# facebookresearch/localrf

Hardware: AMD Instinct MI355X
Metric: rays/sec (4096-ray batch, 512 samples, 300^3 grid) (higher is better)
Workload: dtype f32 (colour network: split-bf16 3-term products on v_mfma_f32_32x32x16_bf16, fp32 accumulate, <= 3e-5 vs the exact-fp32 engine; gathers and compositing fp32); 1 GPU; configs[1]: single 300^3 TensorVMSplit, 4096 rays x 512 samples per GPU, full density+appearance+MLP render, eval forward; rays_per_gpu=4096, samples_per_ray=512, grid=300, parallelism=ray-shard x1, mlp_engine=bf16x3

## Files before the change

### localrf_amd/csrc/lrf_common.h

```cpp
#pragma once
#include "lrf_tu.h"
#include <hip/hip_runtime.h>
#include <stdint.h>
#include "../../include/lrf.h"

namespace lrf {

constexpr int MAT0[3] = {0, 0, 1};
constexpr int MAT1[3] = {1, 2, 2};
constexpr int VEC[3]  = {2, 1, 0};

constexpr int LRF_CAS = 32;
__host__ __device__ constexpr int app_pc(int c) { return 8 * (c / 6) + c % 6; }

constexpr int IMG_BAS  = 0;
constexpr int IMG_W1   = IMG_BAS + 2 * 3 * 64 * 8;
constexpr int IMG_W2   = IMG_W1 + 8 * 2 * 64 * 4;
constexpr int IMG_W3H  = IMG_W2 + 8 * 8 * 64 * 4;
constexpr int IMG_B1   = IMG_W3H + 4 * 32 * 4;
constexpr int IMG_B2   = IMG_B1 + 128;
constexpr int IMG_W3V  = IMG_B2 + 128;
constexpr int IMG_FLOATS = IMG_W3V + 16;

constexpr int IMGB_BAS = 0;
// ... 42 lines not shown
  L.mlp = off; off = align64(off + IMG_FLOATS);
  L.mlpb = off; off = align64(off + (size_t)IMGB_ALL * 4);
  for (int p = 0; p < 3; ++p) { L.aplane2[p] = off; off = align64(off + (size_t)L.pw[p] * L.ph[p] * LRF_CA); }
  for (int p = 0; p < 3; ++p) { L.aline2[p]  = off; off = align64(off + (size_t)L.ll[p] * LRF_CA); }
  L.mlpw = off; off = align64(off + (size_t)W32_ALL_U4 * 4);
  L.mlpwt = off; off = align64(off + (size_t)W32T_ALL_U4 * 4);
  L.total = off;
  return L;
}

constexpr int ACT_FEAT = 0, ACT_LD = 32;
constexpr int GRD_GO = 0, GRD_DFEAT = 16, GRD_DX = 48, GRD_LD = 128;
static_assert(ACT_FEAT % 16 == 0 && ACT_LD % 16 == 0, "fragment blocks are 16 columns");
static_assert(GRD_DFEAT % 16 == 0 && GRD_DX % 16 == 0 && GRD_LD % 16 == 0 && GRD_LD - GRD_DX == 80, "fragment blocks are 16 columns");
__host__ __device__ inline size_t frag_off(size_t row, int col, int ld) {
  return (row >> 4) * (size_t)(16 * ld) + (size_t)((col >> 4) * 256 + ((((col >> 2) & 3) * 16 + (int)(row & 15)) << 2) + (col & 3));
}
__device__ __forceinline__ float* frag_lane_base(float* buf, size_t tile, int ld, int s, int g) {
  return buf + tile * (size_t)(16 * ld) + ((g * 16 + s) << 2);
}
__device__ __forceinline__ const float* grd_dx_row(const float* grd, size_t row) {
  return grd + (row >> 4) * (size_t)(16 * GRD_LD) + GRD_DX * 16 + (row & 15) * (GRD_LD - GRD_DX);
}
__device__ __forceinline__ const float* grd_dx8(const float* grd, size_t row, int p, int grp) {
  return grd + (row >> 4) * (size_t)(16 * GRD_LD) + GRD_DX * 16 + (((p * 3 + grp) * 16 + (int)(row & 15)) << 3);
}

struct DField {
  const float* dplane[3]; const float* dline[3];
  const float* aplane[3]; const float* aline[3];
  const float* mlp;
  const uint4* mlpb;
  const float* aplane2[3]; const float* aline2[3];
  const uint4* mlpw;
  const uint4* mlpwt;
  int pw[3], ph[3], ll[3];
  const float* alpha_vol; int ax, ay, az;
  float m_lo[3], m_inv[3];
  float lo[3], inv[3];
  float hi[3];
  float density_shift, distance_scale, weight_thres;
  float term_T;
  const float* basis; const float* w1; const float* b1; const float* w2; const float* b2;
  const float* w3; const float* b3;
  int fea_pe, view_pe, fc;
  float* dump;
  float* rdir;
  const int* perm;
};

__device__ __forceinline__ void contract3(float& x, float& y, float& z) {
  float m = fmaxf(fmaxf(fabsf(x), fabsf(y)), fabsf(z));
  m = fmaxf(m, 1e-6f);
  if (m > 1.0f) {
    const float s = (2.0f * m - 1.0f) / (m * m);
    x *= s; y *= s; z *= s;
  }
}

__device__ __forceinline__ void tap1d(float u, int size, int& i0, int& i1, float& t) {
  float ix = ((u + 1.0f) * 0.5f) * (float)(size - 1);
  ix = fminf(fmaxf(ix, 0.0f), (float)(size - 1));
  const float f0 = floorf(ix);
  t = ix - f0;
  i0 = (int)f0;
  i1 = min(i0 + 1, size - 1);
}

struct AxisTaps { int i0[3], i1[3]; float t[3]; };
__device__ __forceinline__ AxisTaps axis_taps(const int pw0, const int ph0, const int ll0, const float u[3]) {
  AxisTaps a;
  tap1d(u[0], pw0, a.i0[0], a.i1[0], a.t[0]);
  tap1d(u[1], ph0, a.i0[1], a.i1[1], a.t[1]);
  tap1d(u[2], ll0, a.i0[2], a.i1[2], a.t[2]);
  return a;
}

__device__ __forceinline__ float feature2density(float f, float shift, bool relu) {
  if (relu) return fmaxf(f, 0.0f);
  const float y = f + shift;
  return y > 20.0f ? y : log1pf(expf(y));
}

__device__ __forceinline__ float alpha_mask_sample(const DField& f, float x, float y, float z) {
  const float ux = (x - f.m_lo[0]) * f.m_inv[0] - 1.0f;
  const float uy = (y - f.m_lo[1]) * f.m_inv[1] - 1.0f;
  const float uz = (z - f.m_lo[2]) * f.m_inv[2] - 1.0f;
  const float ix = ((ux + 1.0f) * 0.5f) * (float)(f.ax - 1);
  const float iy = ((uy + 1.0f) * 0.5f) * (float)(f.ay - 1);
  const float iz = ((uz + 1.0f) * 0.5f) * (float)(f.az - 1);
  const float fx = floorf(ix), fy = floorf(iy), fz = floorf(iz);
  const float tx = ix - fx, ty = iy - fy, tz = iz - fz;
  const int x0 = (int)fx, y0 = (int)fy, z0 = (int)fz;
  float out = 0.0f;
#pragma unroll
  for (int dz = 0; dz < 2; ++dz)
#pragma unroll
    for (int dy = 0; dy < 2; ++dy)
#pragma unroll
      for (int dx = 0; dx < 2; ++dx) {
        const int xi = x0 + dx, yi = y0 + dy, zi = z0 + dz;
        if (xi >= 0 && xi < f.ax && yi >= 0 && yi < f.ay && zi >= 0 && zi < f.az) {
          const float w = (dx ? tx : 1.0f - tx) * (dy ? ty : 1.0f - ty) * (dz ? tz : 1.0f - tz);
          out += f.alpha_vol[((size_t)zi * f.ay + yi) * f.ax + xi] * w;
        }
      }
  return out;
}

__device__ __forceinline__ void sample_point(const DField& f, const float o[3], const float dh[3],
                                             float zk, float x[3], float u[3]) {
  x[0] = o[0] + dh[0] * zk; x[1] = o[1] + dh[1] * zk; x[2] = o[2] + dh[2] * zk;
  contract3(x[0], x[1], x[2]);
#pragma unroll
  for (int a = 0; a < 3; ++a) u[a] = (x[a] - f.lo[a]) * f.inv[a] - 1.0f;
}

__device__ __forceinline__ float4 ld4(const float* p) { return *reinterpret_cast<const float4*>(p); }
__device__ __forceinline__ float2 ld2(const float* p) { return *reinterpret_cast<const float2*>(p); }

__device__ __forceinline__ float density_feature(const DField& f, const float u[3]) {
  float feat = 0.0f;
#pragma unroll
  for (int p = 0; p < 3; ++p) {
    int x0, x1, y0, y1, l0, l1; float tx, ty, tl;
    tap1d(u[MAT0[p]], f.pw[p], x0, x1, tx);
    tap1d(u[MAT1[p]], f.ph[p], y0, y1, ty);
    tap1d(u[VEC[p]],  f.ll[p], l0, l1, tl);
    const float* pl = f.dplane[p];
    const float* q00 = pl + ((size_t)y0 * f.pw[p] + x0) * LRF_CD;
    const float* q10 = pl + ((size_t)y0 * f.pw[p] + x1) * LRF_CD;
    const float* q01 = pl + ((size_t)y1 * f.pw[p] + x0) * LRF_CD;
    const float* q11 = pl + ((size_t)y1 * f.pw[p] + x1) * LRF_CD;
    const float* r0 = f.dline[p] + (size_t)l0 * LRF_CD;
    const float* r1 = f.dline[p] + (size_t)l1 * LRF_CD;
    const float w00 = (1.0f - tx) * (1.0f - ty), w10 = tx * (1.0f - ty);
    const float w01 = (1.0f - tx) * ty,          w11 = tx * ty;
    const float wl0 = 1.0f - tl, wl1 = tl;
    float sp = 0.0f;
#pragma unroll
    for (int h = 0; h < LRF_CD / 4; ++h) {
      const float4 a = ld4(q00 + 4 * h), b = ld4(q10 + 4 * h), c = ld4(q01 + 4 * h), d = ld4(q11 + 4 * h);
      const float4 e = ld4(r0 + 4 * h), g = ld4(r1 + 4 * h);
      sp += (a.x * w00 + b.x * w10 + c.x * w01 + d.x * w11) * (e.x * wl0 + g.x * wl1);
      sp += (a.y * w00 + b.y * w10 + c.y * w01 + d.y * w11) * (e.y * wl0 + g.y * wl1);
      sp += (a.z * w00 + b.z * w10 + c.z * w01 + d.z * w11) * (e.z * wl0 + g.z * wl1);
      sp += (a.w * w00 + b.w * w10 + c.w * w01 + d.w * w11) * (e.w * wl0 + g.w * wl1);
    }
    feat += sp;
  }
  return feat;
}

__device__ __forceinline__ float4 ld4b(const float* base, unsigned byte_off) {
  return *reinterpret_cast<const float4*>(reinterpret_cast<const char*>(base) + byte_off);
}

__device__ __forceinline__ float density_feature32(const DField& f, const float u[3]) {
  float feat = 0.0f;
#pragma unroll
  for (int p = 0; p < 3; ++p) {
    int x0, x1, y0, y1, l0, l1; float tx, ty, tl;
    tap1d(u[MAT0[p]], f.pw[p], x0, x1, tx);
    tap1d(u[MAT1[p]], f.ph[p], y0, y1, ty);
    tap1d(u[VEC[p]],  f.ll[p], l0, l1, tl);
    const unsigned row0 = (unsigned)y0 * (unsigned)f.pw[p], row1 = (unsigned)y1 * (unsigned)f.pw[p];
    const unsigned o00 = (row0 + x0) * (LRF_CD * 4u), o10 = (row0 + x1) * (LRF_CD * 4u);
    const unsigned o01 = (row1 + x0) * (LRF_CD * 4u), o11 = (row1 + x1) * (LRF_CD * 4u);
    const unsigned q0 = (unsigned)l0 * (LRF_CD * 4u), q1 = (unsigned)l1 * (LRF_CD * 4u);
    const float w00 = (1.0f - tx) * (1.0f - ty), w10 = tx * (1.0f - ty);
    const float w01 = (1.0f - tx) * ty,          w11 = tx * ty;
    const float wl0 = 1.0f - tl, wl1 = tl;
    float sp = 0.0f;
#pragma unroll
    for (int h = 0; h < LRF_CD / 4; ++h) {
      const float4 a = ld4b(f.dplane[p], o00 + 16 * h), b = ld4b(f.dplane[p], o10 + 16 * h);
      const float4 c = ld4b(f.dplane[p], o01 + 16 * h), d = ld4b(f.dplane[p], o11 + 16 * h);
      const float4 e = ld4b(f.dline[p], q0 + 16 * h), g = ld4b(f.dline[p], q1 + 16 * h);
      sp += (a.x * w00 + b.x * w10 + c.x * w01 + d.x * w11) * (e.x * wl0 + g.x * wl1);
      sp += (a.y * w00 + b.y * w10 + c.y * w01 + d.y * w11) * (e.y * wl0 + g.y * wl1);
      sp += (a.z * w00 + b.z * w10 + c.z * w01 + d.z * w11) * (e.z * wl0 + g.z * wl1);
      sp += (a.w * w00 + b.w * w10 + c.w * w01 + d.w * w11) * (e.w * wl0 + g.w * wl1);
    }
    feat += sp;
  }
  return feat;
}

typedef float f32x2 __attribute__((ext_vector_type(2)));
template <bool LDSL>
__device__ __forceinline__ float density_feature_m(const DField& f, const float u[3], const float* const s_line[3]) {
  f32x2 acc = {0.0f, 0.0f};
  const AxisTaps at = axis_taps(f.pw[0], f.ph[0], f.ll[0], u);
#pragma unroll
  for (int p = 0; p < 3; ++p) {
    const int x0 = at.i0[MAT0[p]], x1 = at.i1[MAT0[p]], y0 = at.i0[MAT1[p]], y1 = at.i1[MAT1[p]];
    const int l0 = at.i0[VEC[p]], l1 = at.i1[VEC[p]];
    const float tx = at.t[MAT0[p]], ty = at.t[MAT1[p]], tl = at.t[VEC[p]];
    const unsigned row0 = (unsigned)y0 * (unsigned)f.pw[p], row1 = (unsigned)y1 * (unsigned)f.pw[p];
    const unsigned o00 = (row0 + x0) * (LRF_CD * 4u), o10 = (row0 + x1) * (LRF_CD * 4u);
    const unsigned o01 = (row1 + x0) * (LRF_CD * 4u), o11 = (row1 + x1) * (LRF_CD * 4u);
    const f32x2 w00 = {(1.0f - tx) * (1.0f - ty), (1.0f - tx) * (1.0f - ty)}, w10 = {tx * (1.0f - ty), tx * (1.0f - ty)};
    const f32x2 w01 = {(1.0f - tx) * ty, (1.0f - tx) * ty}, w11 = {tx * ty, tx * ty};
    const f32x2 wl0 = {1.0f - tl, 1.0f - tl}, wl1 = {tl, tl};
#pragma unroll
    for (int h = 0; h < LRF_CD / 4; ++h) {
      const float4 a = ld4b(f.dplane[p], o00 + 16 * h), b = ld4b(f.dplane[p], o10 + 16 * h);
      const float4 c = ld4b(f.dplane[p], o01 + 16 * h), d = ld4b(f.dplane[p], o11 + 16 * h);
      float4 e, g;
      if (LDSL) {
        e = *reinterpret_cast<const float4*>(s_line[p] + l0 * LRF_CD + 4 * h);
        g = *reinterpret_cast<const float4*>(s_line[p] + l1 * LRF_CD + 4 * h);
      } else {
        e = ld4b(f.dline[p], (unsigned)l0 * (LRF_CD * 4u) + 16 * h);
        g = ld4b(f.dline[p], (unsigned)l1 * (LRF_CD * 4u) + 16 * h);
      }
      const f32x2 a0 = {a.x, a.y}, a1 = {a.z, a.w}, b0 = {b.x, b.y}, b1 = {b.z, b.w};
      const f32x2 c0 = {c.x, c.y}, c1 = {c.z, c.w}, d0 = {d.x, d.y}, d1 = {d.z, d.w};
      const f32x2 e0 = {e.x, e.y}, e1 = {e.z, e.w}, g0 = {g.x, g.y}, g1 = {g.z, g.w};
      acc += (a0 * w00 + b0 * w10 + c0 * w01 + d0 * w11) * (e0 * wl0 + g0 * wl1);
      acc += (a1 * w00 + b1 * w10 + c1 * w01 + d1 * w11) * (e1 * wl0 + g1 * wl1);
    }
  }
  return acc.x + acc.y;
}

__device__ __forceinline__ void wave_scan_prod(float v, int lane, float& excl, float& total) {
  float p = v;
#pragma unroll
  for (int d = 1; d < 64; d <<= 1) {
    const float t = __shfl_up(p, d, 64);
    if (lane >= d) p *= t;
  }
  excl = __shfl_up(p, 1, 64);
  if (lane == 0) excl = 1.0f;
  total = __shfl(p, 63, 64);
}

__device__ __forceinline__ float wave_sum(float v) {
#pragma unroll
  for (int d = 32; d >= 1; d >>= 1) v += __shfl_xor(v, d, 64);
  return v;
}

}
```

### localrf_amd/csrc/lrf_render.hip

```cpp
#include <hip/hip_runtime.h>
#include <stdint.h>
#include <stdio.h>
#include <string.h>
#include <stdlib.h>
#include <mutex>
#include "lrf_common.h"

namespace lrf {

constexpr int ITEM = 16;

thread_local char g_err[512] = "";
static int set_err(const char* msg, hipError_t e = hipSuccess) {
  char* slot = lrf_error_slot();
  if (e != hipSuccess) snprintf(slot, 512, "%s: %s", msg, hipGetErrorString(e));
  else snprintf(slot, 512, "%s", msg);
  return 1;
}
#define LRF_HIP(call) do { hipError_t e_ = (call); if (e_ != hipSuccess) return set_err(#call, e_); } while (0)

struct PackSeg { const float* src; float* dst; int C, H, W, CS, app; };
struct PackTab { PackSeg s[18]; };
struct PackMlp { float* mlp; uint32_t* mlpb; uint32_t* mlpw; uint32_t* mlpwt; int mode; };
__device__ void pack_mlp_elem(const LrfParams& p, float* __restrict__ img, int idx);
// ... 116 lines not shown
    return;
  }
  const int u4 = idx >> 2, wj = idx & 3;
  const int lane = u4 & 63, part = (u4 >> 6) & 1, frag = u4 >> 7;
  const int i = lane & 15, g = lane >> 4;
  unsigned short out[2];
#pragma unroll
  for (int h = 0; h < 2; ++h) {
    const int j = 2 * wj + h;
    float v = 0.0f;
    if (frag < 6) {
      const int t1 = frag / 3, pl = frag % 3, row = 16 * t1 + i;
      if (j < 6 && row < LRF_APP_DIM) v = p.basis[row * 72 + pl * LRF_CA + 6 * g + j];
    } else if (frag < 14) {
      const int t1 = frag - 6;
      const int col = 16 * (j >> 2) + 4 * g + (j & 3);
      if (col < LRF_APP_DIM) v = p.w1[(16 * t1 + i) * LRF_APP_DIM + col];
    } else {
      const int t1 = (frag - 14) >> 2, ks = (frag - 14) & 3;
      const int col = 16 * (2 * ks + (j >> 2)) + 4 * g + (j & 3);
      v = p.w2[(16 * t1 + i) * LRF_FEATC + col];
    }
    const unsigned short hi = bf16_bits(v);
    out[h] = part ? bf16_bits(v - bf16_val(hi)) : hi;
  }
  img[idx] = (uint32_t)out[0] | ((uint32_t)out[1] << 16);
}

__device__ void pack_mlp_w32_elem(const LrfParams& p, uint32_t* __restrict__ img, int idx) {
  if (idx >= W32_ALL_U4 * 4) return;
  if (idx >= W32_U4 * 4) {
    const int e = idx - W32_U4 * 4;
    float v = 0.0f;
    if (e < W32_T_B2) v = p.b1[e - W32_T_B1];
    else if (e < W32_T_W3) v = p.b2[e - W32_T_B2];
    else if (e < W32_T_B3) {
      const int c = (e - W32_T_W3) / W32_T_W3_LD, u = (e - W32_T_W3) % W32_T_W3_LD;
      if (u < LRF_FEATC + 3) v = p.w3[c * (LRF_FEATC + 3) + u];
    } else if (e < W32_T_B3 + 3) v = p.b3[e - W32_T_B3];
    img[idx] = __float_as_uint(v);
    return;
  }
  const int u4 = idx >> 2, wj = idx & 3;
  const int lane = u4 & 63, part = (u4 >> 6) & 1, frag = u4 >> 7;
  const int n = lane & 31, h = lane >> 5;
  unsigned short out[2];
#pragma unroll
  for (int hh = 0; hh < 2; ++hh) {
    const int j = 2 * wj + hh;
    float v = 0.0f;
    if (frag < W32_W1) {
      const int c = w32_chan(h, 8 * frag + j);
      if (c >= 0 && n < LRF_APP_DIM) v = p.basis[n * 72 + c];
    } else if (frag < W32_W2) {
      const int e = frag - W32_W1, m = e >> 1, q = e & 1;
      const int u = w32_unit(0, q, h, j);
      if (u < LRF_APP_DIM) v = p.w1[(32 * m + n) * LRF_APP_DIM + u];
    } else {
      const int e = frag - W32_W2, m = e >> 3, m0 = (e >> 1) & 3, q = e & 1;
      v = p.w2[(32 * m + n) * LRF_FEATC + w32_unit(m0, q, h, j)];
    }
    const unsigned short hi = bf16_bits(v);
    out[hh] = part ? bf16_bits(v - bf16_val(hi)) : hi;
  }
  img[idx] = (uint32_t)out[0] | ((uint32_t)out[1] << 16);
}

constexpr int LRF_MULTI_MAX = 4;
struct MultiF { DField f[LRF_MULTI_MAX]; int nf, Rf, Rs, lo; };
__device__ __forceinline__ int multi_io(const MultiF& m, int k, int vray) { return k * m.Rs + m.lo + (vray - k * m.Rf); }
template <bool MULTI> struct FieldArg { typedef DField type; };
template <> struct FieldArg<true> { typedef MultiF type; };
__device__ __forceinline__ const DField& field_of(const DField& f, int) { return f; }
__device__ __forceinline__ const DField& field_of(const MultiF& m, int k) { return m.f[k]; }

template <bool LDSL, bool MULTI = false>
__global__ __launch_bounds__(1024) void k_march(
    typename FieldArg<MULTI>::type fin, const float* __restrict__ rays, const float* __restrict__ z, int R, int S,
    uint32_t flags, float floater,
    float* __restrict__ depth, float* __restrict__ acc_ws, float* __restrict__ w_all,
    int* __restrict__ ncomp, uint16_t* __restrict__ cidx, float* __restrict__ cw,
    float* __restrict__ feat_out ) {
  extern __shared__ float s_alpha_all[];
  const int wave = threadIdx.x >> 6, lane = threadIdx.x & 63;
  const int nb = gridDim.x;
  const int lb = (nb % 8 == 0) ? (int)(blockIdx.x % 8) * (nb / 8) + (int)(blockIdx.x / 8) : (int)blockIdx.x;
  const int nw = blockDim.x >> 6;
  const int ray = lb * nw + wave;
  int fk_ = 0;
  if constexpr (MULTI) fk_ = min((lb * nw) / fin.Rf, fin.nf - 1);
  const DField& f = field_of(fin, fk_);
  int io_ray = ray;
  if constexpr (MULTI) io_ray = multi_io(fin, fk_, ray);
  const float* s_line[3] = {nullptr, nullptr, nullptr};
  if (LDSL) {
    float* base = s_alpha_all + (size_t)nw * S;
#pragma unroll
    for (int p = 0; p < 3; ++p) {
      const int n = f.ll[p] * LRF_CD / 4;
      float4* dst = reinterpret_cast<float4*>(base);
      const float4* src = reinterpret_cast<const float4*>(f.dline[p]);
      for (int i = threadIdx.x; i < n; i += blockDim.x) dst[i] = src[i];
      s_line[p] = base;
      base += f.ll[p] * LRF_CD;
    }
    __syncthreads();
  }
  if (ray >= R) return;
  float* s_alpha = s_alpha_all + (size_t)wave * S;
  const int oray = f.perm ? f.perm[ray] : io_ray;

  const float* rp = rays + (size_t)io_ray * 6;
  const float o[3] = {rp[0], rp[1], rp[2]};
  const float dn = sqrtf(rp[3] * rp[3] + rp[4] * rp[4] + rp[5] * rp[5]);
  const float dh[3] = {rp[3] / dn, rp[4] / dn, rp[5] / dn};
  const bool relu = flags & LRF_FLAG_RELU_DENS;
  const int nchunk = (S + 63) >> 6;

  {
    float carry = 1.0f;
    bool live = true;
    for (int c = 0; c < nchunk; ++c) {
      const int k = (c << 6) + lane;
      float alpha = 0.0f, fk = -INFINITY;
      if (live && k < S - 1) {
        const float zk = z[k];
        float x[3], u[3];
        sample_point(f, o, dh, zk, x, u);
        bool valid = true;
        if (f.alpha_vol) valid = alpha_mask_sample(f, x[0], x[1], x[2]) > 0.0f;
        if (valid) {
          fk = density_feature_m<LDSL>(f, u, s_line);
          const float sigma = feature2density(fk, f.density_shift, relu);
          const float dist = z[k + 1] - zk;
          alpha = 1.0f - expf(-sigma * dist * f.distance_scale);
        }
      }
      if (k < S) {
        s_alpha[k] = alpha;
        if (feat_out) feat_out[(size_t)ray * S + k] = fk;
      }
      if (live && f.term_T > 0.0f) {
        float v = (k < S - 1) ? (1.0f - alpha + 1e-10f) : 1.0f;
#pragma unroll
        for (int d = 32; d >= 1; d >>= 1) v *= __shfl_xor(v, d, 64);
        carry *= v;
        if (__builtin_amdgcn_readfirstlane(__float_as_int(carry)) < __float_as_int(f.term_T)) live = false;
      }
    }
  }

  float acc = 0.0f, dsum = 0.0f, kbar = 0.0f;
  int nsh = 0;
  const int npass = floater > 0.0f ? 2 : 1;
  for (int pass = 0; pass < npass; ++pass) {
    const bool emit = (pass == npass - 1);
    float carry = 1.0f, a_acc = 0.0f, a_d = 0.0f, a_k = 0.0f;
    for (int c = 0; c < nchunk; ++c) {
      const int k = (c << 6) + lane;
      float alpha = 0.0f;
      if (k < S) {
        alpha = s_alpha[k];
        if (pass == 1 && (float)k < kbar * floater) alpha = 0.0f;
        if (k == S - 1) alpha = 1.0f;
      }
      const float v = (k < S) ? (1.0f - alpha + 1e-10f) : 1.0f;
      float excl, total;
      wave_scan_prod(v, lane, excl, total);
      const float T = carry * excl;
      carry *= total;
      const float w = alpha * T;
      if (pass == 0) {
        a_acc += w;
        a_d += (k < S) ? w * z[k] : 0.0f;
        a_k += w * (float)k;
      }
      if (emit) {
        if (w_all && k < S) w_all[(size_t)oray * S + k] = w;
        const bool sh = (k < S) && (w > f.weight_thres);
        const unsigned long long m = __ballot(sh);
        if (sh) {
          const int pos = nsh + __popcll(m & ((1ull << lane) - 1ull));
          cidx[(size_t)ray * S + pos] = (uint16_t)k;
          cw[(size_t)ray * S + pos] = w;
        }
        nsh += __popcll(m);
      }
    }
    if (pass == 0) {
      acc = wave_sum(a_acc);
      dsum = wave_sum(a_d);
      kbar = wave_sum(a_k);
    }
  }
  if (lane == 0) {
    depth[oray] = dsum / dn;
    acc_ws[ray] = acc;
    ncomp[ray] = nsh;
    if (f.rdir) *reinterpret_cast<float4*>(f.rdir + (size_t)ray * 4) = make_float4(dh[0], dh[1], dh[2], dn);
  }
}

__global__ __launch_bounds__(1024) void k_scan_tiles(const int* __restrict__ ncomp, int R, int* __restrict__ toff) {
  __shared__ int s_wave[16];
  __shared__ int s_carry;
  const int tid = threadIdx.x, lane = tid & 63, wave = tid >> 6;
  if (tid == 0) s_carry = 0;
  __syncthreads();
  for (int base = 0; base < R; base += 1024) {
    const int r = base + tid;
    const int v = r < R ? (ncomp[r] + ITEM - 1) / ITEM : 0;
    int incl = v;
#pragma unroll
    for (int d = 1; d < 64; d <<= 1) {
      const int t = __shfl_up(incl, d, 64);
      if (lane >= d) incl += t;
    }
    if (lane == 63) s_wave[wave] = incl;
    __syncthreads();
    int woff = 0;
    for (int q = 0; q < wave; ++q) woff += s_wave[q];
    const int carry = s_carry;
    if (r < R) toff[r] = carry + woff + incl - v;
    __syncthreads();
    if (tid == 1023) s_carry = carry + woff + incl;
    __syncthreads();
  }
  if (tid == 0) toff[R] = s_carry;
}

typedef float f32x4 __attribute__((ext_vector_type(4)));

__device__ __forceinline__ f32x4 mfma4(float a, float b, f32x4 c) {
  return __builtin_amdgcn_mfma_f32_16x16x4f32(a, b, c, 0, 0, 0);
}

template <int p>
__device__ __forceinline__ void gather_app6_plane(const DField& f, const float u[3], int g, float X[8]) {
  int x0, x1, y0, y1, l0, l1; float tx, ty, tl;
  tap1d(u[MAT0[p]], f.pw[p], x0, x1, tx);
  tap1d(u[MAT1[p]], f.ph[p], y0, y1, ty);
  tap1d(u[VEC[p]],  f.ll[p], l0, l1, tl);
  const float* pl = f.aplane[p] + 8 * g;
  const float* q00 = pl + ((size_t)y0 * f.pw[p] + x0) * LRF_CAS;
  const float* q10 = pl + ((size_t)y0 * f.pw[p] + x1) * LRF_CAS;
  const float* q01 = pl + ((size_t)y1 * f.pw[p] + x0) * LRF_CAS;
  const float* q11 = pl + ((size_t)y1 * f.pw[p] + x1) * LRF_CAS;
  const float* r0 = f.aline[p] + (size_t)l0 * LRF_CAS + 8 * g;
  const float* r1 = f.aline[p] + (size_t)l1 * LRF_CAS + 8 * g;
  const float w00 = (1.0f - tx) * (1.0f - ty), w10 = tx * (1.0f - ty);
  const float w01 = (1.0f - tx) * ty,          w11 = tx * ty;
  const float wl0 = 1.0f - tl, wl1 = tl;
#pragma unroll
  for (int h = 0; h < 2; ++h) {
    const float4 a = ld4(q00 + 4 * h), b = ld4(q10 + 4 * h), c = ld4(q01 + 4 * h), d = ld4(q11 + 4 * h);
    const float4 e = ld4(r0 + 4 * h), q = ld4(r1 + 4 * h);
    X[4 * h]     = (a.x * w00 + b.x * w10 + c.x * w01 + d.x * w11) * (e.x * wl0 + q.x * wl1);
    X[4 * h + 1] = (a.y * w00 + b.y * w10 + c.y * w01 + d.y * w11) * (e.y * wl0 + q.y * wl1);
    X[4 * h + 2] = (a.z * w00 + b.z * w10 + c.z * w01 + d.z * w11) * (e.z * wl0 + q.z * wl1);
    X[4 * h + 3] = (a.w * w00 + b.w * w10 + c.w * w01 + d.w * w11) * (e.w * wl0 + q.w * wl1);
  }
}
__device__ __forceinline__ void gather_app6(const DField& f, const float u[3], int g, float X[3][6]) {
  float v[8];
  gather_app6_plane<0>(f, u, g, v);
#pragma unroll
  for (int j = 0; j < 6; ++j) X[0][j] = v[j];
  gather_app6_plane<1>(f, u, g, v);
#pragma unroll
  for (int j = 0; j < 6; ++j) X[1][j] = v[j];
  gather_app6_plane<2>(f, u, g, v);
#pragma unroll
  for (int j = 0; j < 6; ++j) X[2][j] = v[j];
}

struct TileWalk {
  int t, t_end, ray, next_off;
};
// ... 354 lines not shown
}

struct Workspace {
  int* toff; int* ncomp; float* acc; uint16_t* cidx; float* cw; float* part;
  float* rdir;
  int* perm; float* rays_s;
  int pmax; size_t bytes;
};
static size_t up256(size_t x) { return (x + 255) & ~size_t(255); }
static Workspace carve(void* ws, int R, int S) {
  Workspace w;
  char* p = reinterpret_cast<char*>(ws);
  size_t off = 0;
  w.pmax = 2 * ((S + ITEM3 - 1) / ITEM3);
  w.toff  = reinterpret_cast<int*>(p + off);       off += up256((size_t)(R + 1) * 4);
  w.ncomp = reinterpret_cast<int*>(p + off);       off += up256((size_t)R * 4);
  w.acc   = reinterpret_cast<float*>(p + off);     off += up256((size_t)R * 4);
  w.cidx  = reinterpret_cast<uint16_t*>(p + off);  off += up256((size_t)R * S * 2);
  w.cw    = reinterpret_cast<float*>(p + off);     off += up256((size_t)R * S * 4);
  w.part  = reinterpret_cast<float*>(p + off);     off += up256((size_t)R * w.pmax * 12);
  w.rdir  = reinterpret_cast<float*>(p + off);     off += up256((size_t)R * 16);
  w.perm  = reinterpret_cast<int*>(p + off);       off += up256((size_t)R * 4);
  w.rays_s = reinterpret_cast<float*>(p + off);    off += up256((size_t)R * 24);
  w.bytes = off;
  return w;
}

static float* g_dump = nullptr;
static int g_no_lds_lines = 0;
static int g_pipe_chunk = 16384;
static int g_no_scene_fuse = 0;

static int device_cus() {
  static int cache[64] = {};
  int dev = 0;
  if (hipGetDevice(&dev) != hipSuccess) return 256;
  int& cus = cache[dev & 63];
  if (!cus) {
    hipDeviceProp_t prop;
    if (hipGetDeviceProperties(&prop, dev) == hipSuccess) cus = prop.multiProcessorCount;
    if (cus <= 0) cus = 256;
  }
  return cus;
}

static int g_bwd_overlap = 1;
struct SideStream { hipStream_t s; hipEvent_t fork, join, app[2], bucket[5]; bool ok, bucket_set; std::mutex mu; };
static SideStream* side_stream() {
  static SideStream tab[64];
  static std::mutex init_mu;
  int dev = 0;
  if (hipGetDevice(&dev) != hipSuccess) return nullptr;
  SideStream& x = tab[dev & 63];
  std::lock_guard<std::mutex> lk(init_mu);
  if (!x.ok) {
    if (hipStreamCreateWithFlags(&x.s, hipStreamNonBlocking) != hipSuccess) return nullptr;
    if (hipEventCreateWithFlags(&x.fork, hipEventDisableTiming) != hipSuccess ||
        hipEventCreateWithFlags(&x.join, hipEventDisableTiming) != hipSuccess ||
        hipEventCreateWithFlags(&x.app[0], hipEventDisableTiming) != hipSuccess ||
        hipEventCreateWithFlags(&x.app[1], hipEventDisableTiming) != hipSuccess) return nullptr;
    for (int q = 0; q < 5; ++q)
      if (hipEventCreateWithFlags(&x.bucket[q], hipEventDisableTiming) != hipSuccess) return nullptr;
    x.bucket_set = false;
    x.ok = true;
  }
  return &x;
}
static hipError_t lds_opt_in();

constexpr int LRF_SORT_MAX_R = 32768;
static bool sorts_rays(int R, uint32_t flags) { return (flags & LRF_FLAG_SORT_RAYS) && R >= 2 && R <= LRF_SORT_MAX_R; }
static const float* sort_rays_if_asked(DField& d, const float* rays, int R, uint32_t flags, const Workspace& w, hipStream_t st) {
  d.perm = nullptr;
  if (!sorts_rays(R, flags)) return rays;
  int N = 2;
  while (N < R) N <<= 1;
  hipLaunchKernelGGL(k_sort_rays, dim3(1), dim3(1024), (size_t)N * 4, st, rays, R, N, w.rays_s, w.perm);
  d.perm = w.perm;
  return w.rays_s;
}

static int march_lds_rays(const int32_t ll[3], int S) {
  if (g_no_lds_lines) return 0;
  const size_t lds_l = (size_t)(ll[0] + ll[1] + ll[2]) * LRF_CD * sizeof(float);
  for (int cand = 4; cand <= 16; cand *= 2)
    if (((size_t)cand * S * sizeof(float) + lds_l) * (16 / cand) <= 156 * 1024) return cand;
  return 0;
}
static void launch_march(const DField& d, const float* rays, const float* z, int R, int S, uint32_t flags, float floater,
                         float* depth, float* acc, float* w_all, int* ncomp, uint16_t* cidx, float* cw, float* feat,
                         hipStream_t st, const MultiF* mf = nullptr) {
  const size_t lds_l = (size_t)(d.ll[0] + d.ll[1] + d.ll[2]) * LRF_CD * sizeof(float);
  const int nw = march_lds_rays(d.ll, S);
  if (nw) {
    const size_t lds = (size_t)nw * S * sizeof(float) + lds_l;
    if (mf) {
      hipLaunchKernelGGL((k_march<true, true>), dim3((R + nw - 1) / nw), dim3(64 * nw), lds, st,
                         *mf, rays, z, R, S, flags, floater, depth, acc, w_all, ncomp, cidx, cw, feat);
      return;
    }
    hipLaunchKernelGGL(k_march<true>, dim3((R + nw - 1) / nw), dim3(64 * nw), lds, st,
                       d, rays, z, R, S, flags, floater, depth, acc, w_all, ncomp, cidx, cw, feat);
  } else {
    hipLaunchKernelGGL(k_march<false>, dim3((R + 3) / 4), dim3(256), (size_t)4 * S * sizeof(float), st,
                       d, rays, z, R, S, flags, floater, depth, acc, w_all, ncomp, cidx, cw, feat);
  }
}

static void launch_shade3(DField d, const float* rays, const float* z, int R, int S, uint32_t flags, const Workspace& w,
                         int* toff32, float* rgb, float* acc_out, const SaveOut3* sv, float* dump, hipStream_t st) {
  const size_t lds_base = (size_t)W32_ALL_U4 * sizeof(uint4) + (size_t)S * sizeof(float);
  const size_t lds_toff = (size_t)(R + 1) * sizeof(int) + (size_t)R * sizeof(unsigned short) + 16;
  const bool in_lds = lds_base + lds_toff + 64 <= 160 * 1024 - 256;
  const dim3 grid(device_cus()), block(512);
  if (sv) {
    if (in_lds) {
      hipLaunchKernelGGL((k_shade3<8, true, false, true>), grid, block, lds_base + lds_toff, st,
                         d, rays, z, S, toff32, R, w.ncomp, w.cidx, w.cw, w.part, w.pmax, flags, w.acc, rgb, acc_out, *sv);
    } else {
      hipLaunchKernelGGL(k_scan_tiles_n<ITEM3>, dim3(1), dim3(1024), 0, st, w.ncomp, R, toff32);
      hipLaunchKernelGGL((k_shade3<8, false, false, true>), grid, block, lds_base, st,
                         d, rays, z, S, toff32, R, w.ncomp, w.cidx, w.cw, w.part, w.pmax, flags, w.acc, rgb, acc_out, *sv);
    }
  } else if (in_lds && dump) {
    d.dump = dump;
    hipLaunchKernelGGL((k_shade3<8, true, true>), grid, block, lds_base + lds_toff, st,
                       d, rays, z, S, toff32, R, w.ncomp, w.cidx, w.cw, w.part, w.pmax, flags, w.acc, rgb, acc_out, SaveOut3{});
  } else if (in_lds) {
    hipLaunchKernelGGL((k_shade3<8, true, false>), grid, block, lds_base + lds_toff, st,
                       d, rays, z, S, toff32, R, w.ncomp, w.cidx, w.cw, w.part, w.pmax, flags, w.acc, rgb, acc_out, SaveOut3{});
  } else {
    hipLaunchKernelGGL(k_scan_tiles_n<ITEM3>, dim3(1), dim3(1024), 0, st, w.ncomp, R, toff32);
    hipLaunchKernelGGL((k_shade3<8, false, false>), grid, block, lds_base, st,
                       d, rays, z, S, toff32, R, w.ncomp, w.cidx, w.cw, w.part, w.pmax, flags, w.acc, rgb, acc_out, SaveOut3{});
  }
}

static void launch_shade3_multi(const MultiF& mf, const float* rays, const float* z, int Rv, int S, uint32_t flags,
                                const Workspace& w, float* rgb, hipStream_t st) {
  const size_t lds_base = (size_t)W32_ALL_U4 * sizeof(uint4) + (size_t)S * sizeof(float);
  hipLaunchKernelGGL(k_scan_tiles_n<ITEM3>, dim3(1), dim3(1024), 0, st, w.ncomp, Rv, w.toff);
  hipLaunchKernelGGL((k_shade3m<8, false>), dim3(device_cus()), dim3(512), lds_base, st,
                     mf, rays, z, S, w.toff, Rv, w.ncomp, w.cidx, w.cw, w.part, w.pmax, flags, w.acc, rgb, (float*)nullptr, SaveOut3{});
}

}

#include "lrf_generic.inl"
namespace lrf {
static const char* gen_check(const LrfField* f) {
  const int fc = f->feature_c ? f->feature_c : LRF_FEATC;
  if (f->fea_pe < 0 || f->fea_pe > GEN_MAX_PE || f->view_pe < 0 || f->view_pe > GEN_MAX_PE || fc < 1 || fc > GEN_MAX_FC)
    return "localrf: unsupported colour-network configuration (need 0 <= fea_pe, view_pe <= 6 and 1 <= featureC <= 256)";
  if (!gen_is_default(f->fea_pe, f->view_pe, fc) && (!f->basis || !f->w1 || !f->b1 || !f->w2 || !f->b2 || !f->w3 || !f->b3))
    return "localrf: a non-default colour-network configuration needs the natural-layout weights in LrfField (basis, w1 .. b3)";
  return nullptr;
}
static hipError_t launch_shade_gen(const DField& d, const GenCfg& gc, const float* rays, const float* z, int R, int S, const Workspace& w,
                                   const int* toff32, float* crgb, float* act, int4* tileinfo, hipStream_t st) {
  constexpr int ls = 32;
  const int nt = gen_block_threads(gc);
  const size_t lds = (size_t)gen_lds(gc, ls, false).total * 4;
  const dim3 grid(R * ((w.pmax * 16 + ls - 1) / ls));
  if (toff32) hipLaunchKernelGGL((k_shade_gen<32, true>), grid, dim3(nt), lds, st, d, gc, rays, z, S, w.ncomp, w.cidx, w.cw, w.part, w.pmax, toff32, crgb, act, tileinfo);
  else        hipLaunchKernelGGL((k_shade_gen<32, false>), grid, dim3(nt), lds, st, d, gc, rays, z, S, w.ncomp, w.cidx, w.cw, w.part, w.pmax, toff32, crgb, act, tileinfo);
  return hipGetLastError();
}
}
#include "lrf_backward.inl"
namespace lrf {
static hipError_t lds_opt_in() {
  constexpr int L160 = 160 * 1024;
  static const struct { const void* k; int bytes; } tab[] = {
    {reinterpret_cast<const void*>(&k_sort_rays), LRF_SORT_MAX_R * 4},
    {reinterpret_cast<const void*>(&k_march<true>), L160},
    {reinterpret_cast<const void*>(&k_march<true, true>), L160},
    {reinterpret_cast<const void*>(&k_shade3<8, true, false>), L160 - 256},
    {reinterpret_cast<const void*>(&k_shade3<8, false, false>), L160 - 256},
    {reinterpret_cast<const void*>(&k_shade3<8, true, true>), L160 - 256},
    {reinterpret_cast<const void*>(&k_shade3<8, true, false, true>), L160 - 256},
    {reinterpret_cast<const void*>(&k_shade3<8, false, false, true>), L160 - 256},
    {reinterpret_cast<const void*>(&k_shade3m<8, false>), L160 - 256},
    {reinterpret_cast<const void*>(&k_shade_gen<32, false>), L160 - 1024},
    {reinterpret_cast<const void*>(&k_shade_gen<32, true>), L160 - 1024},
    {reinterpret_cast<const void*>(&k_gen_dgrad<32>), L160 - 1024},
    {reinterpret_cast<const void*>(&k_gen_dgrad<16>), L160 - 1024},
    {reinterpret_cast<const void*>(&k_scatter_plane<LRF_CA, true, LRF_APP_NT, false>), L160},
    {reinterpret_cast<const void*>(&k_scatter_plane<LRF_CA, true, LRF_APP_NT, true>), L160},
    {reinterpret_cast<const void*>(&k_scatter_plane<LRF_CD, false, 512, true>), L160},
    {reinterpret_cast<const void*>(&k_scatter_line<LRF_CA, true, 1024>), L160},
    {reinterpret_cast<const void*>(&k_scatter_line<LRF_CD, false, 1024>), L160},
    {reinterpret_cast<const void*>(&k_bwd_ray), 14 * LRF_MAX_S_TRAIN * 4 + BIN_MAX * 4},
    {reinterpret_cast<const void*>(&k_train_dgrad3<8>), L160 - 256},
    {reinterpret_cast<const void*>(&k_train_app3<8, false>), 128 * 1024},
    {reinterpret_cast<const void*>(&k_train_app3<8, true>), 128 * 1024},
    {reinterpret_cast<const void*>(&k_scatter_fix<LRF_CD, false, FIX_NT>), L160},
    {reinterpret_cast<const void*>(&k_scatter_fix<LRF_CA, true, FIX_NT>), L160},
    {reinterpret_cast<const void*>(&k_scatter_fix<LRF_CA, true, FIX_NT, 4>), L160},
    {reinterpret_cast<const void*>(&k_scatter_det<LRF_CD, false, FIX_NT>), L160},
    {reinterpret_cast<const void*>(&k_scatter_det<LRF_CA, true, FIX_NT>), L160},
    {reinterpret_cast<const void*>(&k_scatter_det<LRF_CA, true, FIX_NT, 4>), L160},
    {reinterpret_cast<const void*>(&k_wgrad_w2w3<128>), (int)w23_lds(128)},
    {reinterpret_cast<const void*>(&k_wgrad_w2w3<64>), (int)w23_lds(64)},
  };
  static std::once_flag once[64];
  static hipError_t err[64];
  int dev = 0;
  const hipError_t e0 = hipGetDevice(&dev);
  if (e0 != hipSuccess) return e0;
  std::call_once(once[dev & 63], [dev] {
    hipError_t e = hipSuccess;
    for (const auto& t : tab)
      if (e == hipSuccess) e = hipFuncSetAttribute(t.k, hipFuncAttributeMaxDynamicSharedMemorySize, t.bytes);
    err[dev & 63] = e;
  });
  return err[dev & 63];
}
}
#include "lrf_scene.inl"
#include "lrf_adam.inl"
#include "lrf_losses.inl"
#include "lrf_metrics.inl"
#include "lrf_frames.inl"
#include "lrf_select.inl"
#include "lrf_evalgeo.inl"
#include "lrf_encode.inl"
#include "lrf_points.inl"
#include "lrf_reg.inl"
#include "lrf_mask.inl"

using namespace lrf;

extern "C" {

int lrf_abi_version(void) { return LRF_ABI_VERSION; }
void lrf_debug_set_dump(float* buf) { g_dump = buf; }
void lrf_debug_set_bwd_overlap(int on) { g_bwd_overlap = (on & 1) ? 1 : 0; if (on > 1) g_wgrad_split = (on >> 1) - 1; }
void lrf_debug_set_lds_lines(int on) { g_no_lds_lines = on ? 0 : 1; }
void lrf_debug_set_pipe_chunk(int rays) { g_pipe_chunk = rays > 0 ? rays : 0; }
#ifdef LRF_SCATTER_PROF
int lrf_debug_scatter_prof(unsigned long long* host_out ) {
  return (int)hipMemcpyFromSymbol(host_out, HIP_SYMBOL(lrf::g_scat_prof), sizeof(unsigned long long) * 2 * 2048 * 12);
}
#endif
void lrf_debug_set_scene_fuse(int on) { g_no_scene_fuse = on ? 0 : 1; }
int64_t lrf_debug_saved_row_offset(int buffer, uint64_t row, int col) {
  using namespace lrf;
  if (buffer == 0) return (col < 0 || col >= ACT_LD) ? -1 : (int64_t)frag_off((size_t)row, col, ACT_LD);
  if (buffer == 1) {
    if (col < 0 || col >= GRD_LD) return -1;
    if (col >= GRD_DX) return (int64_t)((row >> 4) * (uint64_t)(16 * GRD_LD) + GRD_DX * 16 + (row & 15) * (GRD_LD - GRD_DX) + (col - GRD_DX));
    return (int64_t)frag_off((size_t)row, col, GRD_LD);
  }
  return -1;
}
const char* lrf_last_error(void) { return lrf_error_slot(); }
char* lrf_error_slot(void) { return g_err; }

size_t lrf_cache_bytes(const int32_t grid[3]) { return make_layout(grid).total * sizeof(float); }
// ... 264 lines not shown
```

Baseline: 24.50 million rays/s.

## Batch density plane loads, stage z in LDS, mark ray values wave-uniform in march

Restructures density_feature_m so all plane tap loads are issued up front behind a scheduling barrier, then line loads, with packed FMA accumulation. This exposes more memory-level parallelism. It also caches the z sample array in LDS per block, marks per-ray direction and carry values as wave-uniform via readfirstlane, and replaces the predicated alpha-mask gather with clamped unconditional loads. In exchange it raises register pressure from holding all taps live, which may lower occupancy, and adds LDS use for z.

```diff
diff --git a/localrf_amd/csrc/lrf_common.h b/localrf_amd/csrc/lrf_common.h
--- a/localrf_amd/csrc/lrf_common.h
+++ b/localrf_amd/csrc/lrf_common.h
@@ -148,29 +148,32 @@
   return y > 20.0f ? y : log1pf(expf(y));
 }
 
+__device__ __forceinline__ float wave_uniform(float v) { return __int_as_float(__builtin_amdgcn_readfirstlane(__float_as_int(v))); }
+
 __device__ __forceinline__ float alpha_mask_sample(const DField& f, float x, float y, float z) {
   const float ux = (x - f.m_lo[0]) * f.m_inv[0] - 1.0f;
   const float uy = (y - f.m_lo[1]) * f.m_inv[1] - 1.0f;
   const float uz = (z - f.m_lo[2]) * f.m_inv[2] - 1.0f;
-  const float ix = ((ux + 1.0f) * 0.5f) * (float)(f.ax - 1);
-  const float iy = ((uy + 1.0f) * 0.5f) * (float)(f.ay - 1);
-  const float iz = ((uz + 1.0f) * 0.5f) * (float)(f.az - 1);
-  const float fx = floorf(ix), fy = floorf(iy), fz = floorf(iz);
-  const float tx = ix - fx, ty = iy - fy, tz = iz - fz;
+  const float hx = (ux + 1.0f) * 0.5f, hy = (uy + 1.0f) * 0.5f, hz = (uz + 1.0f) * 0.5f;
+  const float sx = wave_uniform((float)(f.ax - 1)), sy = wave_uniform((float)(f.ay - 1)), sz = wave_uniform((float)(f.az - 1));
+  const float fx = floorf(hx * sx), fy = floorf(hy * sy), fz = floorf(hz * sz);
+  const float tx = fmaf(hx, sx, -fx), ty = fmaf(hy, sy, -fy), tz = fmaf(hz, sz, -fz);
   const int x0 = (int)fx, y0 = (int)fy, z0 = (int)fz;
+  float vol[8];
+  bool inb[8];
+#pragma unroll
+  for (int t = 0; t < 8; ++t) {
+    const int xi = x0 + (t & 1), yi = y0 + ((t >> 1) & 1), zi = z0 + (t >> 2);
+    inb[t] = xi >= 0 && xi < f.ax && yi >= 0 && yi < f.ay && zi >= 0 && zi < f.az;
+    const int xc = min(max(xi, 0), f.ax - 1), yc = min(max(yi, 0), f.ay - 1), zc = min(max(zi, 0), f.az - 1);
+    vol[t] = f.alpha_vol[((size_t)zc * f.ay + yc) * f.ax + xc];
+  }
   float out = 0.0f;
 #pragma unroll
-  for (int dz = 0; dz < 2; ++dz)
-#pragma unroll
-    for (int dy = 0; dy < 2; ++dy)
-#pragma unroll
-      for (int dx = 0; dx < 2; ++dx) {
-        const int xi = x0 + dx, yi = y0 + dy, zi = z0 + dz;
-        if (xi >= 0 && xi < f.ax && yi >= 0 && yi < f.ay && zi >= 0 && zi < f.az) {
-          const float w = (dx ? tx : 1.0f - tx) * (dy ? ty : 1.0f - ty) * (dz ? tz : 1.0f - tz);
-          out += f.alpha_vol[((size_t)zi * f.ay + yi) * f.ax + xi] * w;
-        }
-      }
+  for (int t = 0; t < 8; ++t) {
+    const float w = ((t & 1) ? tx : 1.0f - tx) * (((t >> 1) & 1) ? ty : 1.0f - ty) * ((t >> 2) ? tz : 1.0f - tz);
+    out = inb[t] ? fmaf(vol[t], w, out) : out;
+  }
   return out;
 }
 
@@ -254,38 +257,79 @@
 }
 
 typedef float f32x2 __attribute__((ext_vector_type(2)));
+__device__ __forceinline__ f32x2 pk_fma(f32x2 a, f32x2 b, f32x2 c) { return __builtin_elementwise_fma(a, b, c); }
 template <bool LDSL>
 __device__ __forceinline__ float density_feature_m(const DField& f, const float u[3], const float* const s_line[3]) {
-  f32x2 acc = {0.0f, 0.0f};
-  const AxisTaps at = axis_taps(f.pw[0], f.ph[0], f.ll[0], u);
+  AxisTaps at;
+  const int gs[3] = {f.pw[0], f.ph[0], f.ll[0]};
+#pragma unroll
+  for (int a = 0; a < 3; ++a) {
+    const float sm1 = wave_uniform((float)(gs[a] - 1));
+    float ix = ((u[a] + 1.0f) * 0.5f) * sm1;
+    ix = fminf(fmaxf(ix, 0.0f), sm1);
+    const float f0 = floorf(ix);
+    at.t[a] = ix - f0;
+    at.i0[a] = (int)f0;
+    at.i1[a] = min(at.i0[a] + 1, gs[a] - 1);
+  }
+  unsigned o[3][4];
 #pragma unroll
   for (int p = 0; p < 3; ++p) {
     const int x0 = at.i0[MAT0[p]], x1 = at.i1[MAT0[p]], y0 = at.i0[MAT1[p]], y1 = at.i1[MAT1[p]];
-    const int l0 = at.i0[VEC[p]], l1 = at.i1[VEC[p]];
-    const float tx = at.t[MAT0[p]], ty = at.t[MAT1[p]], tl = at.t[VEC[p]];
     const unsigned row0 = (unsigned)y0 * (unsigned)f.pw[p], row1 = (unsigned)y1 * (unsigned)f.pw[p];
-    const unsigned o00 = (row0 + x0) * (LRF_CD * 4u), o10 = (row0 + x1) * (LRF_CD * 4u);
-    const unsigned o01 = (row1 + x0) * (LRF_CD * 4u), o11 = (row1 + x1) * (LRF_CD * 4u);
+    o[p][0] = (row0 + x0) * (LRF_CD * 4u); o[p][1] = (row0 + x1) * (LRF_CD * 4u);
+    o[p][2] = (row1 + x0) * (LRF_CD * 4u); o[p][3] = (row1 + x1) * (LRF_CD * 4u);
+  }
+  float4 t[3][4][LRF_CD / 4], ln[3][2][LRF_CD / 4];
+#pragma unroll
+  for (int p = 0; p < 3; ++p)
+#pragma unroll
+    for (int j = 0; j < 4; ++j)
+#pragma unroll
+      for (int h = 0; h < LRF_CD / 4; ++h) t[p][j][h] = ld4b(f.dplane[p], o[p][j] + 16 * h);
+  __builtin_amdgcn_sched_barrier(0);
+  f32x2 pv[3][LRF_CD / 2];
+#pragma unroll
+  for (int p = 0; p < 3; ++p) {
+    const float tx = at.t[MAT0[p]], ty = at.t[MAT1[p]];
     const f32x2 w00 = {(1.0f - tx) * (1.0f - ty), (1.0f - tx) * (1.0f - ty)}, w10 = {tx * (1.0f - ty), tx * (1.0f - ty)};
     const f32x2 w01 = {(1.0f - tx) * ty, (1.0f - tx) * ty}, w11 = {tx * ty, tx * ty};
-    const f32x2 wl0 = {1.0f - tl, 1.0f - tl}, wl1 = {tl, tl};
-#pragma unroll
-    for (int h = 0; h < LRF_CD / 4; ++h) {
-      const float4 a = ld4b(f.dplane[p], o00 + 16 * h), b = ld4b(f.dplane[p], o10 + 16 * h);
-      const float4 c = ld4b(f.dplane[p], o01 + 16 * h), d = ld4b(f.dplane[p], o11 + 16 * h);
-      float4 e, g;
-      if (LDSL) {
-        e = *reinterpret_cast<const float4*>(s_line[p] + l0 * LRF_CD + 4 * h);
-        g = *reinterpret_cast<const float4*>(s_line[p] + l1 * LRF_CD + 4 * h);
-      } else {
-        e = ld4b(f.dline[p], (unsigned)l0 * (LRF_CD * 4u) + 16 * h);
-        g = ld4b(f.dline[p], (unsigned)l1 * (LRF_CD * 4u) + 16 * h);
-      }
+#pragma unroll
+    for (int h = 0; h < LRF_CD / 4; ++h) {
+      const float4 a = t[p][0][h], b = t[p][1][h], c = t[p][2][h], d = t[p][3][h];
       const f32x2 a0 = {a.x, a.y}, a1 = {a.z, a.w}, b0 = {b.x, b.y}, b1 = {b.z, b.w};
       const f32x2 c0 = {c.x, c.y}, c1 = {c.z, c.w}, d0 = {d.x, d.y}, d1 = {d.z, d.w};
+      pv[p][2 * h]     = pk_fma(d0, w11, pk_fma(c0, w01, pk_fma(a0, w00, b0 * w10)));
+      pv[p][2 * h + 1] = pk_fma(d1, w11, pk_fma(c1, w01, pk_fma(a1, w00, b1 * w10)));
+    }
+  }
+  if (!LDSL) __builtin_amdgcn_sched_barrier(0);
+#pragma unroll
+  for (int p = 0; p < 3; ++p) {
+    const int l0 = at.i0[VEC[p]], l1 = at.i1[VEC[p]];
+#pragma unroll
+    for (int h = 0; h < LRF_CD / 4; ++h) {
+      if (LDSL) {
+        ln[p][0][h] = *reinterpret_cast<const float4*>(s_line[p] + l0 * LRF_CD + 4 * h);
+        ln[p][1][h] = *reinterpret_cast<const float4*>(s_line[p] + l1 * LRF_CD + 4 * h);
+      } else {
+        ln[p][0][h] = ld4b(f.dline[p], (unsigned)l0 * (LRF_CD * 4u) + 16 * h);
+        ln[p][1][h] = ld4b(f.dline[p], (unsigned)l1 * (LRF_CD * 4u) + 16 * h);
+      }
+    }
+  }
+  if (!LDSL) __builtin_amdgcn_sched_barrier(0);
+  f32x2 acc = {0.0f, 0.0f};
+#pragma unroll
+  for (int p = 0; p < 3; ++p) {
+    const float tl = at.t[VEC[p]];
+    const f32x2 wl0 = {1.0f - tl, 1.0f - tl}, wl1 = {tl, tl};
+#pragma unroll
+    for (int h = 0; h < LRF_CD / 4; ++h) {
+      const float4 e = ln[p][0][h], g = ln[p][1][h];
       const f32x2 e0 = {e.x, e.y}, e1 = {e.z, e.w}, g0 = {g.x, g.y}, g1 = {g.z, g.w};
-      acc += (a0 * w00 + b0 * w10 + c0 * w01 + d0 * w11) * (e0 * wl0 + g0 * wl1);
-      acc += (a1 * w00 + b1 * w10 + c1 * w01 + d1 * w11) * (e1 * wl0 + g1 * wl1);
+      acc = pk_fma(pv[p][2 * h], pk_fma(e0, wl0, g0 * wl1), acc);
+      acc = pk_fma(pv[p][2 * h + 1], pk_fma(e1, wl0, g1 * wl1), acc);
     }
   }
   return acc.x + acc.y;
diff --git a/localrf_amd/csrc/lrf_render.hip b/localrf_amd/csrc/lrf_render.hip
--- a/localrf_amd/csrc/lrf_render.hip
+++ b/localrf_amd/csrc/lrf_render.hip
@@ -222,7 +222,7 @@
     int* __restrict__ ncomp, uint16_t* __restrict__ cidx, float* __restrict__ cw,
     float* __restrict__ feat_out ) {
   extern __shared__ float s_alpha_all[];
-  const int wave = threadIdx.x >> 6, lane = threadIdx.x & 63;
+  const int wave = __builtin_amdgcn_readfirstlane(threadIdx.x >> 6), lane = threadIdx.x & 63;
   const int nb = gridDim.x;
   const int lb = (nb % 8 == 0) ? (int)(blockIdx.x % 8) * (nb / 8) + (int)(blockIdx.x / 8) : (int)blockIdx.x;
   const int nw = blockDim.x >> 6;
@@ -233,8 +233,8 @@
   int io_ray = ray;
   if constexpr (MULTI) io_ray = multi_io(fin, fk_, ray);
   const float* s_line[3] = {nullptr, nullptr, nullptr};
+  float* base = s_alpha_all + (size_t)nw * S;
   if (LDSL) {
-    float* base = s_alpha_all + (size_t)nw * S;
 #pragma unroll
     for (int p = 0; p < 3; ++p) {
       const int n = f.ll[p] * LRF_CD / 4;
@@ -244,16 +244,18 @@
       s_line[p] = base;
       base += f.ll[p] * LRF_CD;
     }
-    __syncthreads();
-  }
+  }
+  float* s_z = base;
+  for (int i = threadIdx.x; i < S; i += blockDim.x) s_z[i] = z[i];
+  __syncthreads();
   if (ray >= R) return;
   float* s_alpha = s_alpha_all + (size_t)wave * S;
   const int oray = f.perm ? f.perm[ray] : io_ray;
 
   const float* rp = rays + (size_t)io_ray * 6;
   const float o[3] = {rp[0], rp[1], rp[2]};
-  const float dn = sqrtf(rp[3] * rp[3] + rp[4] * rp[4] + rp[5] * rp[5]);
-  const float dh[3] = {rp[3] / dn, rp[4] / dn, rp[5] / dn};
+  const float dn = wave_uniform(sqrtf(rp[3] * rp[3] + rp[4] * rp[4] + rp[5] * rp[5]));
+  const float dh[3] = {wave_uniform(rp[3] / dn), wave_uniform(rp[4] / dn), wave_uniform(rp[5] / dn)};
   const bool relu = flags & LRF_FLAG_RELU_DENS;
   const int nchunk = (S + 63) >> 6;
 
@@ -264,7 +266,7 @@
       const int k = (c << 6) + lane;
       float alpha = 0.0f, fk = -INFINITY;
       if (live && k < S - 1) {
-        const float zk = z[k];
+        const float zk = s_z[k];
         float x[3], u[3];
         sample_point(f, o, dh, zk, x, u);
         bool valid = true;
@@ -272,24 +274,25 @@
         if (valid) {
           fk = density_feature_m<LDSL>(f, u, s_line);
           const float sigma = feature2density(fk, f.density_shift, relu);
-          const float dist = z[k + 1] - zk;
+          const float dist = s_z[k + 1] - s_z[k];
           alpha = 1.0f - expf(-sigma * dist * f.distance_scale);
         }
       }
       if (k < S) {
         s_alpha[k] = alpha;
-        if (feat_out) feat_out[(size_t)ray * S + k] = fk;
+        if (feat_out) (feat_out + (size_t)ray * S)[(unsigned)k] = fk;
       }
       if (live && f.term_T > 0.0f) {
         float v = (k < S - 1) ? (1.0f - alpha + 1e-10f) : 1.0f;
 #pragma unroll
         for (int d = 32; d >= 1; d >>= 1) v *= __shfl_xor(v, d, 64);
-        carry *= v;
-        if (__builtin_amdgcn_readfirstlane(__float_as_int(carry)) < __float_as_int(f.term_T)) live = false;
-      }
-    }
-  }
-
+        carry = wave_uniform(carry * v);
+        if (__float_as_int(carry) < __float_as_int(f.term_T)) live = false;
+      }
+    }
+  }
+
+  const int lane_b = __lane_id();
   float acc = 0.0f, dsum = 0.0f, kbar = 0.0f;
   int nsh = 0;
   const int npass = floater > 0.0f ? 2 : 1;
@@ -297,7 +300,7 @@
     const bool emit = (pass == npass - 1);
     float carry = 1.0f, a_acc = 0.0f, a_d = 0.0f, a_k = 0.0f;
     for (int c = 0; c < nchunk; ++c) {
-      const int k = (c << 6) + lane;
+      const int k = (c << 6) + lane_b;
       float alpha = 0.0f;
       if (k < S) {
         alpha = s_alpha[k];
@@ -306,13 +309,13 @@
       }
       const float v = (k < S) ? (1.0f - alpha + 1e-10f) : 1.0f;
       float excl, total;
-      wave_scan_prod(v, lane, excl, total);
+      wave_scan_prod(v, lane_b, excl, total);
       const float T = carry * excl;
       carry *= total;
       const float w = alpha * T;
       if (pass == 0) {
         a_acc += w;
-        a_d += (k < S) ? w * z[k] : 0.0f;
+        a_d += (k < S) ? w * s_z[k] : 0.0f;
         a_k += w * (float)k;
       }
       if (emit) {
@@ -320,7 +323,7 @@
         const bool sh = (k < S) && (w > f.weight_thres);
         const unsigned long long m = __ballot(sh);
         if (sh) {
-          const int pos = nsh + __popcll(m & ((1ull << lane) - 1ull));
+          const int pos = nsh + __popcll(m & ((1ull << lane_b) - 1ull));
           cidx[(size_t)ray * S + pos] = (uint16_t)k;
           cw[(size_t)ray * S + pos] = w;
         }
@@ -333,7 +336,7 @@
       kbar = wave_sum(a_k);
     }
   }
-  if (lane == 0) {
+  if (lane_b == 0) {
     depth[oray] = dsum / dn;
     acc_ws[ray] = acc;
     ncomp[ray] = nsh;
@@ -854,7 +857,7 @@
 
 static int march_lds_rays(const int32_t ll[3], int S) {
   if (g_no_lds_lines) return 0;
-  const size_t lds_l = (size_t)(ll[0] + ll[1] + ll[2]) * LRF_CD * sizeof(float);
+  const size_t lds_l = (size_t)(ll[0] + ll[1] + ll[2]) * LRF_CD * sizeof(float) + (size_t)S * sizeof(float);
   for (int cand = 4; cand <= 16; cand *= 2)
     if (((size_t)cand * S * sizeof(float) + lds_l) * (16 / cand) <= 156 * 1024) return cand;
   return 0;
@@ -862,7 +865,7 @@
 static void launch_march(const DField& d, const float* rays, const float* z, int R, int S, uint32_t flags, float floater,
                          float* depth, float* acc, float* w_all, int* ncomp, uint16_t* cidx, float* cw, float* feat,
                          hipStream_t st, const MultiF* mf = nullptr) {
-  const size_t lds_l = (size_t)(d.ll[0] + d.ll[1] + d.ll[2]) * LRF_CD * sizeof(float);
+  const size_t lds_l = (size_t)(d.ll[0] + d.ll[1] + d.ll[2]) * LRF_CD * sizeof(float) + (size_t)S * sizeof(float);
   const int nw = march_lds_rays(d.ll, S);
   if (nw) {
     const size_t lds = (size_t)nw * S * sizeof(float) + lds_l;
@@ -874,7 +877,7 @@
     hipLaunchKernelGGL(k_march<true>, dim3((R + nw - 1) / nw), dim3(64 * nw), lds, st,
                        d, rays, z, R, S, flags, floater, depth, acc, w_all, ncomp, cidx, cw, feat);
   } else {
-    hipLaunchKernelGGL(k_march<false>, dim3((R + 3) / 4), dim3(256), (size_t)4 * S * sizeof(float), st,
+    hipLaunchKernelGGL(k_march<false>, dim3((R + 3) / 4), dim3(256), (size_t)5 * S * sizeof(float), st,
                        d, rays, z, R, S, flags, floater, depth, acc, w_all, ncomp, cidx, cw, feat);
   }
 }
@@ -947,6 +950,7 @@
     {reinterpret_cast<const void*>(&k_sort_rays), LRF_SORT_MAX_R * 4},
     {reinterpret_cast<const void*>(&k_march<true>), L160},
     {reinterpret_cast<const void*>(&k_march<true, true>), L160},
+    {reinterpret_cast<const void*>(&k_march<false>), L160},
     {reinterpret_cast<const void*>(&k_shade3<8, true, false>), L160 - 256},
     {reinterpret_cast<const void*>(&k_shade3<8, false, false>), L160 - 256},
     {reinterpret_cast<const void*>(&k_shade3<8, true, true>), L160 - 256},
```

Result: no change. 24.43 million rays/s, median of 2 (-0.3%).
